# Gryph66/gymwipe

Hardware: AMD Instinct MI355X
Metric: env.step()/s at 65 536 parallel envs, counter-traffic band-assign (higher is better)
Workload: dtype f64

## Files before the change

### gymwipe_amd/csrc/ct_rollout_sfx.hip

```cpp
#include "ct_common.hip.h"
#include "gw_dispatch.h"
#include "gw_queue.h"

using namespace gwk;

namespace {


constexpr int TP_ENVS = 64, TP_STEPS = 64;

__global__ __launch_bounds__(256) void pack_actions_kernel(uint32_t N, int K, int Kp, const int32_t* __restrict__ device,
                                                           const int32_t* __restrict__ duration, uint16_t* __restrict__ packed)
{
    __shared__ __attribute__((aligned(16))) uint16_t tile[TP_ENVS][TP_STEPS + 2];
    const uint32_t e0 = blockIdx.x * TP_ENVS;
    const int t = threadIdx.x;
    const bool vec_ok = (N & 3u) == 0;
    for (int k0 = 0; k0 < Kp; k0 += TP_STEPS) {
        const int c4 = (t & 15) * 4, r = t >> 4;
#pragma unroll
        for (int pass = 0; pass < TP_STEPS / 16; ++pass) {
            const int kk = pass * 16 + r, k = k0 + kk;
            uint32_t v[4] = {0xffffu, 0xffffu, 0xffffu, 0xffffu};
            if (k < K) {
// ... 132 lines not shown
    }
    {
        const int n_tr = (R * R * S + 15) >> 4, n_be = (2 * D * S * 8) >> 4, n_cl = (2 * D * S) >> 4;
        for (int i = threadIdx.x; i < n_tr; i += blockDim.x) *reinterpret_cast<uint4*>(s_trans + ((uint32_t)i << 4)) = ld<uint4>(st.trans, (uint32_t)i << 4);
        for (int i = threadIdx.x; i < n_be; i += blockDim.x) *reinterpret_cast<uint4*>(reinterpret_cast<uint8_t*>(s_ber) + ((uint32_t)i << 4)) = ld<uint4>(st.ber2, (uint32_t)i << 4);
        for (int i = threadIdx.x; i < n_cl; i += blockDim.x) *reinterpret_cast<uint4*>(s_cls + ((uint32_t)i << 4)) = ld<uint4>(st.cls2, (uint32_t)i << 4);
    }
    __syncthreads();
    if (e >= N) return;

    const uint32_t RB = GEN ? (uint32_t)st.RB : 16u * NWC;
    const uint32_t o16 = e << 4, oq = e * RB;
    const uint4 ip = ld<uint4>(st.ip, o16);
    const double2 tw = ld<double2>(st.tw, o16);
    const uint4 tk = ld<uint4>(st.tk, o16);
    typename ArrSel<GEN, DM>::rw len, tb;
    typename ArrSel<GEN, DM + 1>::rw sta;
    if constexpr (GEN) {
        uint32_t* col = s_cols + (threadIdx.x & 63);
        len.p = col; tb.p = col + DM * 64; sta.p = col + 2 * DM * 64;
        for (int i = 0; i < D; ++i) len[i] = st.qb[oq + (uint32_t)i];
        for (int j = 0; j < R; ++j) sta[j] = st.qb[oq + (uint32_t)(D + j)];
    } else {
        uint4 qw[NWC];
#pragma unroll
        for (int w = 0; w < NWC; ++w) qw[w] = ld<uint4>(st.qb, oq + 16u * w);
#pragma unroll
        for (int i = 0; i < DT; ++i) len[i] = (word_of(qw[i >> 4], (i >> 2) & 3) >> ((i & 3) * 8)) & 0xffu;
#pragma unroll
        for (int j = 0; j < DT + 1; ++j) sta[j] = (word_of(qw[(DT + j) >> 4], ((DT + j) >> 2) & 3) >> (((DT + j) & 3) * 8)) & 0xffu;
    }
    double now = tw.x, wake = tw.y;
    uint32_t tau = tk.x;
    const uint32_t nbp = tk.y;
    GwBp bpc, bpp;
    bpc.t0 = ip.x; bpc.c0 = ip.y;
    bpp.t0 = ip.z; bpp.c0 = ip.w;
    const GwBp* hist = st.bph + ((size_t)e << 7);
    uint32_t rvm = tk.z;
    int32_t last_abs = (int32_t)(tk.w & 0x7fffffffu);
    uint32_t dn = tk.w >> 31;

    constexpr bool FAST = MODE >= 1, NOLIM = MODE == 2;
    const StepMathT<FAST, NOLIM> m(c);
    const double slot = c.slot, br = c.bit_rate, hd = c.hdr_dur, hdr_bits = c.hdr_bits, interval = c.counter_interval;
    const double inv_interval = c.inv_interval, tie_filter = c.tie_filter;
    const bool fast_ticks = FAST || c.fast_ticks != 0;
    const uint32_t bound = (uint32_t)c.counter_bound, base_bytes = (uint32_t)(c.mac_hdr + c.net_hdr);
    const int mh = c.mac_hdr, pv = c.payload_value;
    uint32_t live_mask = 0u;
    if constexpr (GEN) {
        for (int i = 0; i < D; ++i) live_mask |= ((s_term[i] >> sta[i]) & 1u) ? 0u : (1u << i);
    }
    typename ArrSel<GEN, DM>::ro mult, term, inv16;
    if constexpr (GEN) {
        mult.p = st.cst->mult; mult.shift16 = 0; term.p = st.cst->term; term.shift16 = 1; inv16.p = st.cst->inv16; inv16.shift16 = 0;
// ... 206 lines not shown
            len_d = gw_len_after_ticks(len_d, kk, mult_d, kt);
        }
    }

    {
        uint32_t kk = 0;
        while (wake <= now) { if (wake == now) fl |= GW_FLAG_TIE; wake = wake + interval; kk++; }
        tau += kk;
#pragma unroll
        for (int i = 0; i < D; ++i) len[i] = gw_len_after_ticks(len[i], tau - tb[i], mult[i], kt);
    }

    if constexpr (GEN) {
        for (int i = 0; i < D; ++i) st.qb[oq + (uint32_t)i] = (uint8_t)len[i];
        for (int j = 0; j < R; ++j) st.qb[oq + (uint32_t)(D + j)] = (uint8_t)sta[j];
    } else {
        uint32_t nb[16 * NWC];
#pragma unroll
        for (int b = 0; b < 16 * NWC; ++b) nb[b] = 0u;
#pragma unroll
        for (int i = 0; i < DT; ++i) nb[i] = len[i];
#pragma unroll
        for (int j = 0; j < DT + 1; ++j) nb[DT + j] = sta[j];
#pragma unroll
        for (int w = 0; w < NWC; ++w) {
            const int b = 16 * w;
            uint4 o;
            o.x = nb[b + 0] | (nb[b + 1] << 8) | (nb[b + 2] << 16) | (nb[b + 3] << 24);
            o.y = nb[b + 4] | (nb[b + 5] << 8) | (nb[b + 6] << 16) | (nb[b + 7] << 24);
            o.z = nb[b + 8] | (nb[b + 9] << 8) | (nb[b + 10] << 16) | (nb[b + 11] << 24);
            o.w = nb[b + 12] | (nb[b + 13] << 8) | (nb[b + 14] << 16) | (nb[b + 15] << 24);
            st_plain(st.qb, oq + 16u * w, o);
        }
    }
    st_plain(st.tw, o16, make_double2(now, wake));
    st_plain(st.tk, o16, make_uint4(tau, nbp, rvm, (uint32_t)last_abs | (dn << 31)));
    publish_env_counters(st.sa, N, e, kt.pop, kt.deliv, k_bad, fl, (uint32_t)K);
}

__device__ __forceinline__ uint32_t gw_policy_u(uint64_t seed, uint64_t env_term, uint64_t step)
{
    uint64_t z = seed ^ env_term ^ (step * 0xD1B54A32D192ED03ull);
    z += 0x9E3779B97F4A7C15ull;
    z = (z ^ (z >> 30)) * 0xBF58476D1CE4E5B9ull;
    z = (z ^ (z >> 27)) * 0x94D049BB133111EBull;
    z ^= z >> 31;
    return gw_min_u32((uint32_t)z, 0xfffffffeu);
}
template <class ROW>
__device__ __forceinline__ uint32_t gw_policy_upper(ROW row, uint32_t A, uint32_t u)
{
// ... 411 lines not shown
```

### gymwipe_amd/csrc/ct_rollout_sync_body.h

```cpp
    constexpr bool GEN = DT == 0;
    constexpr int DM = GEN ? GW_MAX_DEVICES : DT;
    constexpr int NWC = (2 * DM + 1 + 15) / 16;
    constexpr int S = GW_MAX_NSTATES;
    const int D = GEN ? c.D : DT, R = D + 1, RRM = D;
    const uint32_t N = (uint32_t)st.N;
    const uint32_t e = blockIdx.x * blockDim.x + threadIdx.x;

    constexpr int TRANS_B = ((DM + 1) * (DM + 1) * S + 15) / 16 * 16;
    __shared__ __attribute__((aligned(16))) uint8_t s_trans[TRANS_B];
    __shared__ __attribute__((aligned(16))) double  s_ber[2 * DM * S];
    __shared__ __attribute__((aligned(16))) uint8_t s_cls[2 * DM * S];
    __shared__ uint32_t s_cols[GEN ? (3 * DM + 1) * 64 : 1];
    __shared__ uint2 s_mi[GEN ? DM : 1];
    __shared__ uint32_t s_term[GEN ? DM : 1];
    if constexpr (GEN) {
        for (int i = threadIdx.x; i < D; i += blockDim.x) {
            s_mi[i] = make_uint2((uint32_t)st.cst->mult[i], st.cst->inv16[i]);
            s_term[i] = st.cst->term[i];
        }
    }
    {
        const int n_tr = (R * R * S + 15) >> 4, n_be = (2 * D * S * 8) >> 4, n_cl = (2 * D * S) >> 4;
        for (int i = threadIdx.x; i < n_tr; i += blockDim.x) *reinterpret_cast<uint4*>(s_trans + ((uint32_t)i << 4)) = ld<uint4>(st.trans, (uint32_t)i << 4);
        for (int i = threadIdx.x; i < n_be; i += blockDim.x) *reinterpret_cast<uint4*>(reinterpret_cast<uint8_t*>(s_ber) + ((uint32_t)i << 4)) = ld<uint4>(st.ber2, (uint32_t)i << 4);
        for (int i = threadIdx.x; i < n_cl; i += blockDim.x) *reinterpret_cast<uint4*>(s_cls + ((uint32_t)i << 4)) = ld<uint4>(st.cls2, (uint32_t)i << 4);
    }
    GW_ROLLOUT_SRC_STAGE
    __syncthreads();
    if (e >= N) return;

    const uint32_t RB = GEN ? (uint32_t)st.RB : 16u * NWC;
    const uint32_t o16 = e << 4, oq = e * RB;
    const uint4 ip = ld<uint4>(st.ip, o16);
    const double2 tw = ld<double2>(st.tw, o16);
    const uint4 tk = ld<uint4>(st.tk, o16);
    typename ArrSel<GEN, DM>::rw len, tb;
    typename ArrSel<GEN, DM + 1>::rw sta;
    if constexpr (GEN) {
        uint32_t* col = s_cols + (threadIdx.x & 63);
        len.p = col; tb.p = col + DM * 64; sta.p = col + 2 * DM * 64;
        for (int i = 0; i < D; ++i) len[i] = st.qb[oq + (uint32_t)i];
        for (int j = 0; j < R; ++j) sta[j] = st.qb[oq + (uint32_t)(D + j)];
    } else {
        uint4 qw[NWC];
#pragma unroll
        for (int w = 0; w < NWC; ++w) qw[w] = ld<uint4>(st.qb, oq + 16u * w);
#pragma unroll
        for (int i = 0; i < DT; ++i) len[i] = (word_of(qw[i >> 4], (i >> 2) & 3) >> ((i & 3) * 8)) & 0xffu;
#pragma unroll
        for (int j = 0; j < DT + 1; ++j) sta[j] = (word_of(qw[(DT + j) >> 4], ((DT + j) >> 2) & 3) >> (((DT + j) & 3) * 8)) & 0xffu;
    }
    double now = tw.x, wake = tw.y;
    uint32_t tau = tk.x;
    const uint32_t nbp = tk.y;
    GwBp bpc, bpp;
    bpc.t0 = ip.x; bpc.c0 = ip.y;
    bpp.t0 = ip.z; bpp.c0 = ip.w;
    const GwBp* hist = st.bph + ((size_t)e << 7);
    uint32_t rvm = tk.z;
    int32_t last_abs = (int32_t)(tk.w & 0x7fffffffu);
    uint32_t dn = tk.w >> 31;

    constexpr bool FAST = MODE >= 1, NOLIM = MODE == 2;
    const StepMathT<FAST, NOLIM> m(c);
    const double slot = c.slot, br = c.bit_rate, hd = c.hdr_dur, hdr_bits = c.hdr_bits, interval = c.counter_interval;
    const double inv_interval = c.inv_interval, tie_filter = c.tie_filter, coded_factor = c.coded_factor;
    const bool fast_ticks = FAST || c.fast_ticks != 0;
    const bool idem = c.idem_states != 0;
    const uint32_t bound = (uint32_t)c.counter_bound, base_bytes = (uint32_t)(c.mac_hdr + c.net_hdr);
    const int mh = c.mac_hdr, pv = c.payload_value;
    uint32_t live_mask = 0u;
    if constexpr (GEN) {
        for (int i = 0; i < D; ++i) live_mask |= ((s_term[i] >> sta[i]) & 1u) ? 0u : (1u << i);
    }
    typename ArrSel<GEN, DM>::ro mult, term, inv16;
    if constexpr (GEN) {
// ... 237 lines not shown
        uint32_t nb[16 * NWC];
#pragma unroll
        for (int b = 0; b < 16 * NWC; ++b) nb[b] = 0u;
#pragma unroll
        for (int i = 0; i < DT; ++i) nb[i] = len[i];
#pragma unroll
        for (int j = 0; j < DT + 1; ++j) nb[DT + j] = sta[j];
#pragma unroll
        for (int w = 0; w < NWC; ++w) {
            const int b = 16 * w;
            uint4 o;
            o.x = nb[b + 0] | (nb[b + 1] << 8) | (nb[b + 2] << 16) | (nb[b + 3] << 24);
            o.y = nb[b + 4] | (nb[b + 5] << 8) | (nb[b + 6] << 16) | (nb[b + 7] << 24);
            o.z = nb[b + 8] | (nb[b + 9] << 8) | (nb[b + 10] << 16) | (nb[b + 11] << 24);
            o.w = nb[b + 12] | (nb[b + 13] << 8) | (nb[b + 14] << 16) | (nb[b + 15] << 24);
            st_plain(st.qb, oq + 16u * w, o);
        }
    }
    st_plain(st.tw, o16, make_double2(now, wake));
    st_plain(st.tk, o16, make_uint4(tau, nbp, rvm, (uint32_t)last_abs | (dn << 31)));
    publish_env_counters(st.sa, N, e, kt.pop, kt.deliv, k_bad, fl, (uint32_t)K);
```

### gymwipe_amd/csrc/ct_step_sfx.hip

```cpp
#include "ct_common.hip.h"
#include "gw_dispatch.h"
#include "gw_queue.h"

using namespace gwk;


namespace {



#define PIN_V(x) asm volatile("" : "+v"(x))
#define PIN_S(x) asm volatile("" : "+s"(x))

template <int DT, bool FEEDBACK, int MODE, bool HALF = false>
__device__ __forceinline__ void ct_step_sfx_body(const GwState& st, const GwDevConst& c,
                                                 const int32_t* __restrict__ device,
                                                 const int32_t* __restrict__ duration,
                                                 int32_t* __restrict__ obs,
                                                 float* __restrict__ reward,
                                                 uint8_t* __restrict__ done,
                                                 uint8_t* __restrict__ fb,
                                                 int n_stage,
                                                 double& now_out, bool& live_out)
{
    constexpr bool PACKED = DT > 0;
    constexpr bool FAST = MODE >= 1, NOLIM = MODE == 2;
    constexpr int NWC = DT > 0 ? (2 * DT + 1 + 15) / 16 : 1;
    const uint32_t N = (uint32_t)st.N;
    const uint32_t e = HALF ? blockIdx.x * 32u + (threadIdx.x & 31u) : blockIdx.x * 64u + threadIdx.x;
    const int D = DT > 0 ? DT : c.D;
    const int R = D + 1, RRM = D;
    constexpr int S = GW_MAX_NSTATES;
    const uint32_t RB = PACKED ? 16u * NWC : (uint32_t)st.RB;

    STAMP(0);
    constexpr int DM = DT > 0 ? DT : GW_MAX_DEVICES;
    constexpr GwStripeLayout LM(DM);
    const GwStripeLayout L(D);
    constexpr int MAX_CH = LM.staged_chunks(GW_MAX_NSTATES);
    const int n_ch = n_stage < MAX_CH ? n_stage : MAX_CH;
    const int tid = threadIdx.x;
    constexpr int nthr = 64;
// ... 9 lines not shown
            r_ch[i] = ld<uint4>(st.blob, (uint32_t)(ch < n_ch ? ch : 0) << 4);
        }
    }

    Tally k = {0, 0, 0, 0, 0};
    uint32_t k_bad = 0;

    const bool live = e < N && (!HALF || threadIdx.x < 32u);
    const uint32_t el = live ? e : 0u;
    const uint32_t o16 = e << 4, o16l = el << 4;
    const uint32_t oq = e * RB, oql = el * RB;
    int d = device[el];
    int du = duration[el];
    uint4 ip = ld<uint4>(st.ip, o16l);
    const double2 tw = ld<double2>(st.tw, o16l);
    const uint4 tk = ld<uint4>(st.tk, o16l);
    uint4 qw[NWC];
#pragma unroll
    for (int w = 0; w < NWC; ++w) qw[w] = PACKED ? ld<uint4>(st.qb, oql + 16u * w) : make_uint4(0u, 0u, 0u, 0u);
    now_out = tw.x;
    live_out = live;
    if (one_pass) {
#pragma unroll
        for (int i = 0; i < PER; ++i) {
            const int ch = tid + i * nthr;
            *reinterpret_cast<uint4*>(s_blob + ((uint32_t)ch << 4)) = r_ch[i];
        }
    } else {
        for (int i = tid; i < n_ch; i += nthr) *reinterpret_cast<uint4*>(s_blob + ((uint32_t)i << 4)) = ld<uint4>(st.blob, (uint32_t)i << 4);
    }
    STAMP(1);
// ... 16 lines not shown
    PIN_V(d); PIN_V(du);
    PIN_V(ip.x); PIN_V(ip.y); PIN_V(ip.z); PIN_V(ip.w);
    const uint2* s_mi = reinterpret_cast<const uint2*>(s_blob + L.mi);
    const uint8_t* s_st = s_blob + L.s0;
    const uint8_t* g_h2 = st.blob + L.h2;
    const uint32_t STR = (uint32_t)L.stripe, DD = (uint32_t)D;
    auto t_ber0 = [&](uint32_t dd, uint32_t ss) { return *reinterpret_cast<const double*>(s_st + ss * STR + (uint32_t)L.ber0 + dd * 8u); };
    auto t_ber1 = [&](uint32_t dd, uint32_t ss) { return *reinterpret_cast<const double*>(s_st + ss * STR + (uint32_t)L.ber1 + dd * 8u); };
    auto t_h1 = [&](uint32_t j, uint32_t ss) { return (uint32_t)s_st[ss * STR + (uint32_t)L.h1 + j]; };
    auto t_r1 = [&](uint32_t dd, uint32_t ss) { return (uint32_t)s_st[ss * STR + (uint32_t)L.r1 + dd]; };
    auto t_cls0 = [&](uint32_t dd, uint32_t ss) { return (uint32_t)s_st[ss * STR + (uint32_t)L.cls0 + dd]; };
    auto t_cls1 = [&](uint32_t dd, uint32_t ss) { return (uint32_t)s_st[ss * STR + (uint32_t)L.cls1 + dd]; };
    auto t_h2 = [&](uint32_t j, uint32_t dd, uint32_t ss) { return (uint32_t)g_h2[(ss * DD + j) * DD + dd]; };

    if (live) {
        uint32_t rvm = tk.z;
#ifdef GW_STAMPS
        asm volatile("" : "+v"(rvm));
#endif
        STAMP(3);
        int32_t last_abs = (int32_t)(tk.w & 0x7fffffffu);
        uint32_t dn = tk.w >> 31;
        uint32_t fl = 0;

        if ((unsigned)d >= (unsigned)D || (unsigned)du >= (unsigned)max_duration) {
            fl = GW_FLAG_BADACT;
            k_bad = 1;
            const int32_t latest = pv * ((int)(rvm & 1u) - (int)((rvm >> 1) & 1u));
            if (FEEDBACK) {
                obs[e] = latest + cbound;
                reward[e] = 0.0f;
                done[e] = (uint8_t)dn;
                if (fb) fb[e] = (uint8_t)((uint32_t)(((latest > 0) - (latest < 0)) + 1) | (10u << 2) | (dn << 7));
            }
        } else {
            const uint32_t bound = (uint32_t)cbound;
            const uint32_t base_bytes = (uint32_t)base_b;
// ... 15 lines not shown
                        const bool hl = ((uint32_t)d >> 4) == (uint32_t)w, hs = ((uint32_t)(DT + d) >> 4) == (uint32_t)w;
                        lx = hl ? q0 : lx; ly = hl ? q1 : ly; lz = hl ? q2 : lz; lw = hl ? q3 : lw;
                        sx = hs ? q0 : sx; sy = hs ? q1 : sy; sz = hs ? q2 : sz; sw = hs ? q3 : sw;
                    }
                    len_d = byte_of(lx, ly, lz, lw, (uint32_t)d & 15u);
                    s_d_old = byte_of(sx, sy, sz, sw, (uint32_t)(DT + d) & 15u);
                }
                s_r_old = (word_of(qw[(2 * DT) >> 4], ((2 * DT) >> 2) & 3) >> (((2 * DT) & 3) * 8)) & 0xffu;
            } else {
                len_d = st.qb[oq + (uint32_t)d];
                s_d_old = st.qb[oq + (uint32_t)(D + d)];
                s_r_old = st.qb[oq + (uint32_t)(2 * D)];
            }
            const double t_a = tw.x;
            double wake = tw.y;
            const uint32_t tau0 = tk.x, nbp = tk.y;
            GwBp bpc, bpp;
            bpc.t0 = ip.x; bpc.c0 = ip.y;
            bpp.t0 = ip.z; bpp.c0 = ip.w;
            const GwBp* hist = st.bph + ((size_t)e << 7);
            const uint32_t s_d = t_h1((uint32_t)d, s_d_old);
            const uint32_t s_r1 = t_r1((uint32_t)d, s_r_old);
            const uint2 mi = s_mi[d];
            uint32_t nb[PACKED ? 16 * NWC : 1];
            uint32_t n1[PACKED ? DT : 1], n2[PACKED ? DT : 1], mlt[PACKED ? DT : 1];
            if (PACKED) {
#pragma unroll
                for (int b = 0; b < 16 * NWC; ++b) nb[b] = (word_of(qw[b >> 4], (b >> 2) & 3) >> ((b & 3) * 8)) & 0xffu;
#pragma unroll
                for (int i = 0; i < DT; ++i) {
                    n1[i] = t_h1((uint32_t)i, nb[DT + i]);
// ... 116 lines not shown
                    k.deliv += okx ? pops : 0u;
                    rvm |= okx ? (1u << d) : 0u;
                    dn = (okx && pv == cbound) ? 1u : dn;
                }
                if (more)
                for (;;) {
                    if (len_d == 0) {
                        if (mult_d != 0u && wake < stopw) {
                            cur = wake;
                            wake = wake + interval;
                            tau++;
                            len_d = gw_len_after_ticks(0u, 1u, mult_d, kd);
                        } else break;
                    }
                    const uint32_t age = gw_ceil_div(len_d, mult_d, inv16_d);
                    const uint32_t s = base_bytes + gw_tick_value(tau - age, bpc, bpp, nbp, hist, bound);
                    const double need = m.over_rate((double)(s * 8u));
                    if (!((stopw - cur) > need)) break;
                    len_d--;
                    k.pop++;
                    const int pay = (int)s - mh;
                    const TxTimes x = tx_times(m, cur, hd, m.over_rate((double)(pay * 8)));
                    k.tx++;
                    n_data++;
                    double ber_x = ber_x1;
                    uint32_t cls_x = cls_x1;
                    if (idem) {
                        s_r = s_r1;
                    } else {
                        s_r = st.trans[(uint32_t)((RRM * R + d) * S) + s_r];
                        ber_x = st.ber[(uint32_t)((RRM * R + d) * S) + s_r];
// ... 24 lines not shown
                return s;
            };
            if (PACKED) {
                const uint32_t heard_data = n_data ? 0xffffffffu : 0u;
#pragma unroll
                for (int i = 0; i < DT; ++i) {
                    Tally ki = {0, 0, 0, 0, 0};
                    const uint32_t li = gw_len_after_ticks(nb[i], n_ticks, mlt[i], ki);
                    uint32_t si = (n2[i] & heard_data) | (n1[i] & ~heard_data);
                    if (!idem) si = heard_slow(i, nb[DT + i]);
                    if (i != d) { k.app += ki.app; k.drop += ki.drop; }
                    nb[i] = (i == d) ? len_d : li;
                    nb[DT + i] = (i == d) ? s_d : si;
                }
                nb[2 * DT] = s_r;
                uint4 o[NWC];
#pragma unroll
                for (int w = 0; w < NWC; ++w) {
                    const int b = 16 * w;
                    o[w].x = nb[b + 0] | (nb[b + 1] << 8) | (nb[b + 2] << 16) | (nb[b + 3] << 24);
                    o[w].y = nb[b + 4] | (nb[b + 5] << 8) | (nb[b + 6] << 16) | (nb[b + 7] << 24);
                    o[w].z = nb[b + 8] | (nb[b + 9] << 8) | (nb[b + 10] << 16) | (nb[b + 11] << 24);
                    o[w].w = nb[b + 12] | (nb[b + 13] << 8) | (nb[b + 14] << 16) | (nb[b + 15] << 24);
                }
                STAMP(9);
#pragma unroll
                for (int w = 0; w < NWC; ++w) st_(st.qb, oq + 16u * w, o[w]);
            } else {
                for (int i = 0; i < D; ++i) {
                    if (i == d) continue;
                    const uint32_t l0 = st.qb[oq + (uint32_t)i];
                    const uint32_t s0 = st.qb[oq + (uint32_t)(D + i)];
                    const uint32_t s1 = !idem ? heard_slow(i, s0)
                                              : (n_data ? t_h2((uint32_t)i, (uint32_t)d, s0) : t_h1((uint32_t)i, s0));
                    st.qb[oq + (uint32_t)i] = (uint8_t)gw_len_after_ticks(l0, n_ticks, s_mi[i].x, k);
                    if (s1 != s0) st.qb[oq + (uint32_t)(D + i)] = (uint8_t)s1;
                }
                st.qb[oq + (uint32_t)d] = (uint8_t)len_d;
// ... 4 lines not shown
            STAMP(10);
            const int32_t latest = pv * ((int)(rvm & 1u) - (int)((rvm >> 1) & 1u));
            const int32_t abs_d = latest < 0 ? -latest : latest;
            int32_t r = last_abs - abs_d;
            last_abs = abs_d;
            r = r > 10 ? 10 : (r < -10 ? -10 : r);
            if (FEEDBACK) {
                st_(obs, e << 2, (int32_t)(latest + cbound));
                st_(reward, e << 2, (float)r);
                st_(done, e, (uint8_t)dn);
                if (fb) st_(fb, e, (uint8_t)((uint32_t)(((latest > 0) - (latest < 0)) + 1) | ((uint32_t)(r + 10) << 2) | (dn << 7)));
            }
            now_out = t_end;

            st_(st.tw, o16, make_double2(t_end, wake));
            st_(st.tk, o16, make_uint4(tau, nbp, rvm, (uint32_t)last_abs | (dn << 31)));
        }
        STAMP(11);
        publish_env_counters(st.sa, N, e, k.pop, k.deliv, k_bad, fl, 1u);
    }
    STAMP(12);
}

template <int DT, int MODE>
__global__ __launch_bounds__(64) void ct_step_sfx_kernel(GW_LEAD_PARAMS_U64, uint64_t obs_a, uint64_t reward_a, uint64_t done_a, uint64_t fb_a)
{
    uint32_t* __restrict__ ip = gw_global_at<uint32_t>(ip_a);
    double* __restrict__ tw = gw_global_at<double>(tw_a);
    uint32_t* __restrict__ tk = gw_global_at<uint32_t>(tk_a);
    uint8_t* __restrict__ qb = gw_global_at<uint8_t>(qb_a);
    const int32_t* __restrict__ device = gw_global_at<const int32_t>(device_a);
// ... 131 lines not shown
    for (int w = 0; w < GW_SA_WORDS; ++w) st.sa[(size_t)w * st.N + e] = 0u;
    if (e == 0u) { st.sa[(size_t)4 * st.N] = 0u; st.sa[(size_t)4 * st.N + 1] = 0u; }
}

__global__ void ct_reset_sfx_kernel(uint32_t* __restrict__ ip, uint32_t n_envs, uint32_t n_dev, const uint8_t* __restrict__ mask,
                                    int32_t* __restrict__ obs)
{
    const uint32_t e = blockIdx.x * blockDim.x + threadIdx.x;
    if (e >= n_envs) return;
    const uint8_t* base = reinterpret_cast<const uint8_t*>(ip) - gw_blob_header((int)n_dev);
    const GW_AS_CONST GwState* hs = (const GW_AS_CONST GwState*)(base + gw_hdr_st_off((int)n_dev));
    uint32_t* tkp = gw_as_global(hs->tk);
    GwBp* bph = gw_as_global(hs->bph);
    const GW_AS_CONST GwDevConst* c = (const GW_AS_CONST GwDevConst*)(base + gw_hdr_cst_off((int)n_dev));
    const uint32_t o16 = e << 4;
    uint32_t rvm;
    if (!mask || mask[e]) {
        uint4 tk = ld<uint4>(tkp, o16);
        uint4 bp = ld<uint4>(ip, o16);
        GwBp cur; cur.t0 = bp.x; cur.c0 = 0u;
        if (bp.x == tk.x) {
            bph[((size_t)e << 7) + ((tk.y - 1u) & GW_RING_MASK)] = cur;
            bp.y = 0u;
        } else {
            bp.z = bp.x; bp.w = bp.y;
            cur.t0 = tk.x;
            bph[((size_t)e << 7) + (tk.y & GW_RING_MASK)] = cur;
            tk.y += 1u; bp.x = cur.t0; bp.y = 0u;
        }
        tk.z = 0u; tk.w = 0u;
        st_(tkp, o16, tk);
        st_(ip, o16, bp);
        rvm = 0u;
    } else {
        rvm = ld<uint4>(tkp, o16).z;
    }
    if (obs) obs[e] = c->payload_value * ((int)(rvm & 1u) - (int)((rvm >> 1) & 1u)) + c->counter_bound;
}

__global__ void ct_received_sfx_kernel(GwState st, int32_t* __restrict__ out)
{
    const int64_t idx = (int64_t)blockIdx.x * blockDim.x + threadIdx.x;
    const int D = st.D;
    if (idx >= st.N * D) return;
    const uint32_t e = (uint32_t)(idx / D);
    const int i = (int)(idx - (int64_t)e * D);
    const uint32_t rvm = ld<uint4>(st.tk, e << 4).z;
    out[idx] = ((rvm >> i) & 1u) ? st.cst->payload_value : 0;
}

__global__ void ct_delivered_sfx_kernel(GwState st, uint32_t* __restrict__ out)
{
    const uint32_t e = blockIdx.x * blockDim.x + threadIdx.x;
    if (e < (uint32_t)st.N) out[e] = st.sa[(size_t)2 * e + 1];
}

__global__ void ct_clear_flags_kernel(GwState st)
{
    const int64_t e = (int64_t)blockIdx.x * blockDim.x + threadIdx.x;
    if (e < st.N) {
        if (st.sa) st.sa[(size_t)3 * st.N + e] = 0u;
        if (st.xc) st.xc[(size_t)e * 4 + 3] = 0u;
// ... 118 lines not shown
```

### gymwipe_amd/csrc/gw_api.cpp

```cpp
#include "gw_internal.h"
#include "gw_queue.h"
#include "gw_runq.h"
#include "gw_fastmath.h"

#include <hip/hip_runtime.h>

#include <math.h>
#include <stdarg.h>
#include <stdio.h>
#include <stdlib.h>
#include <string.h>
#include <new>
#include <vector>
#include <deque>
#include <atomic>
#include <string>

namespace {

thread_local char g_err[512] = "";

int fail(int code, const char* fmt, ...)
{
    va_list ap;
// ... 210 lines not shown
    for (int j = 0; j < R; ++j) {
        uint16_t m = 0;
        for (int s0 = 0; s0 < tab.nstates[j]; ++s0) {
            bool fixed = true;
            for (int f = 0; f < R && fixed; ++f)
                if (f != j && tab.trans[((size_t)j * R + f) * GW_MAX_NSTATES + s0] != s0) fixed = false;
            if (fixed) m |= (uint16_t)(1u << s0);
        }
        k.term[j] = m;
    }
    return GW_OK;
}

int gw_validate_config(const gw_config& cfg) { return validate(cfg); }

struct GwEnvCounts { std::vector<uint64_t> steps, tx, deliv, app, pop, drop, bad; std::vector<uint32_t> flags; };
static int derive_env_counts(gw_env* env, GwEnvCounts& c)
{
    const GwState& st = env->st;
    const int64_t N = st.N;
    const int D = st.D, RB = st.RB;
    std::vector<uint32_t> sa((size_t)N * GW_SA_WORDS + 2), tk((size_t)N * 4);
    std::vector<uint8_t> qb((size_t)N * RB);
    HIP_TRY(hipMemcpy(sa.data(), st.sa, sa.size() * sizeof(uint32_t), hipMemcpyDeviceToHost));
    HIP_TRY(hipMemcpy(tk.data(), st.tk, tk.size() * sizeof(uint32_t), hipMemcpyDeviceToHost));
    HIP_TRY(hipMemcpy(qb.data(), st.qb, qb.size(), hipMemcpyDeviceToHost));
    uint64_t mult_sum = 0;
    for (int i = 0; i < D; ++i) mult_sum += (uint64_t)env->cfg.mult[i];
    const uint64_t n_steps = (uint64_t)sa[(size_t)4 * N] | ((uint64_t)sa[(size_t)4 * N + 1] << 32);
    c.steps.resize(N); c.tx.resize(N); c.deliv.resize(N); c.app.resize(N); c.pop.resize(N); c.drop.resize(N); c.bad.resize(N);
    c.flags.resize(N);
    for (int64_t e = 0; e < N; ++e) {
        uint64_t queued = 0;
        for (int i = 0; i < D; ++i) queued += qb[(size_t)e * RB + i];
        c.pop[e] = sa[(size_t)2 * e];
        c.deliv[e] = sa[(size_t)2 * e + 1];
        c.bad[e] = sa[(size_t)2 * N + e];
        c.flags[e] = sa[(size_t)3 * N + e];
        c.steps[e] = n_steps - c.bad[e];
        c.tx[e] = c.steps[e] + c.pop[e];
        c.app[e] = (uint64_t)tk[(size_t)e * 4] * mult_sum;
// ... 560 lines not shown
int gw_now_ptr(gw_env* env, const void** now_dev, int64_t* stride_bytes)
{
    if (!env || !now_dev || !stride_bytes) return fail(GW_EINVAL, "env/now/stride is NULL");
    if (env->st.tw) { *now_dev = env->st.tw; *stride_bytes = 16; }
    else { *now_dev = env->st.xw; *stride_bytes = 16; }
    return GW_OK;
}

struct GwSnapHeader {
    uint32_t magic, abi;
    uint64_t total;
    gw_config cfg;
    int32_t nblocks, dyn;
    uint64_t block_bytes[32];
    double t_bound;
    int32_t captured, pad;
};
static const uint32_t kSnapMagic = 0x4e535747u;

int gw_snapshot_bytes(gw_env* env, uint64_t* bytes)
{
    if (!env || !bytes) return fail(GW_EINVAL, "env/bytes is NULL");
    uint64_t t = sizeof(GwSnapHeader);
    for (int i = 0; i < env->nblocks_create; ++i) t += env->block_bytes[i];
    *bytes = t;
    return GW_OK;
}

int gw_get_snapshot(gw_env* env, void* dst, uint64_t bytes)
{
    if (!env || !dst) return fail(GW_EINVAL, "env/dst is NULL");
    uint64_t need = 0;
    int rc = gw_snapshot_bytes(env, &need);
    if (rc) return rc;
    if (bytes != need) return fail(GW_EINVAL, "snapshot needs %llu bytes, got %llu", (unsigned long long)need, (unsigned long long)bytes);
    if ((rc = select_device(env))) return rc;
    HIP_TRY(hipDeviceSynchronize());
    GwSnapHeader h;
    memset(&h, 0, sizeof h);
    h.magic = kSnapMagic; h.abi = GW_ABI_VERSION; h.total = need; h.cfg = env->cfg; h.nblocks = env->nblocks_create; h.dyn = env->dyn;
    for (int i = 0; i < env->nblocks_create; ++i) h.block_bytes[i] = env->block_bytes[i];
    h.t_bound = env->t_bound;
    h.captured = env->captured;
    uint8_t* o = (uint8_t*)dst;
    memcpy(o, &h, sizeof h);
    o += sizeof h;
    for (int i = 0; i < env->nblocks_create; ++i) {
        HIP_TRY(hipMemcpy(o, env->blocks[i], env->block_bytes[i], hipMemcpyDeviceToHost));
        o += env->block_bytes[i];
    }
    return GW_OK;
}

int gw_set_state(gw_env* env, const void* src, uint64_t bytes)
{
    if (!env || !src) return fail(GW_EINVAL, "env/src is NULL");
    uint64_t need = 0;
    int rc = gw_snapshot_bytes(env, &need);
    if (rc) return rc;
    if (bytes != need) return fail(GW_EINVAL, "a snapshot of this handle has %llu bytes, got %llu", (unsigned long long)need, (unsigned long long)bytes);
    GwSnapHeader h;
    memcpy(&h, src, sizeof h);
    if (h.magic != kSnapMagic || h.abi != (uint32_t)GW_ABI_VERSION || h.total != bytes) return fail(GW_EINVAL, "not a snapshot of this ABI");
    gw_config a = h.cfg, b = env->cfg;
    a.hip_device = b.hip_device = 0;
    if (memcmp(&a, &b, sizeof a) != 0 || h.nblocks != env->nblocks_create || h.dyn != env->dyn)
        return fail(GW_EINVAL, "snapshot belongs to a handle with another configuration");
    for (int i = 0; i < h.nblocks; ++i)
        if (h.block_bytes[i] != env->block_bytes[i]) return fail(GW_EINVAL, "snapshot belongs to a handle with another layout");
    if ((rc = select_device(env))) return rc;
    HIP_TRY(hipDeviceSynchronize());
    const uint8_t* in = (const uint8_t*)src + sizeof h;
    for (int i = 0; i < h.nblocks; ++i) {
        HIP_TRY(hipMemcpy(env->blocks[i], in, env->block_bytes[i], hipMemcpyHostToDevice));
        in += env->block_bytes[i];
    }
    if (env->st.ip && (rc = upload_header_structs(env))) return rc;
    env->t_bound = h.t_bound > env->t_bound ? h.t_bound : env->t_bound;
    env->captured |= h.captured;
    HIP_TRY(hipDeviceSynchronize());
    return GW_OK;
}
// ... 282 lines not shown
                    if (k == 5) { NEED(N, uint32_t); memcpy(dst, c.flags.data(), bytes); return GW_OK; }
                    NEED(N, uint64_t);
                    const std::vector<uint64_t>& v = k == 0 ? c.tx : (k == 1 ? c.deliv : (k == 2 ? c.app : (k == 3 ? c.pop : c.drop)));
                    memcpy(dst, v.data(), bytes);
                    return GW_OK;
                }
        }
        const int RB = st.RB;
        std::vector<double> tw((size_t)N * 2);
        std::vector<uint32_t> tk((size_t)N * 4), ip((size_t)N * 4);
        std::vector<uint8_t> qb((size_t)N * RB);
        HIP_TRY(hipMemcpy(tw.data(), st.tw, tw.size() * sizeof(double), hipMemcpyDeviceToHost));
        HIP_TRY(hipMemcpy(tk.data(), st.tk, tk.size() * sizeof(uint32_t), hipMemcpyDeviceToHost));
        HIP_TRY(hipMemcpy(ip.data(), st.ip, ip.size() * sizeof(uint32_t), hipMemcpyDeviceToHost));
        HIP_TRY(hipMemcpy(qb.data(), st.qb, qb.size(), hipMemcpyDeviceToHost));
        const uint32_t bound = (uint32_t)env->cfg.counter_bound;
        const int pv = env->cfg.payload_value;
        if (!strcmp(field, "now")) { NEED(N, double); double* o = (double*)dst; for (int64_t e = 0; e < N; ++e) o[e] = tw[e * 2]; return GW_OK; }
        if (!strcmp(field, "wake")) {
            NEED(N * D, double); double* o = (double*)dst;
            for (int64_t e = 0; e < N; ++e) for (int i = 0; i < D; ++i) o[e * D + i] = tw[e * 2 + 1];
            return GW_OK;
        }
        if (!strcmp(field, "counter")) {
            NEED(N * D, uint32_t); uint32_t* o = (uint32_t*)dst;
            for (int64_t e = 0; e < N; ++e) {
                const uint32_t v = gw_min_u32(ip[e * 4 + 1] + (tk[e * 4] - ip[e * 4]), bound);
                for (int i = 0; i < D; ++i) o[e * D + i] = v;
            }
            return GW_OK;
// ... 148 lines not shown
```

### gymwipe_amd/csrc/gw_queue.h

```cpp
#pragma once
#include <stdint.h>
#include "gw_internal.h"

#if defined(__HIPCC__)
#include <hip/hip_runtime.h>
#define GW_HD __host__ __device__ __forceinline__
#else
#define GW_HD inline
#endif

struct GwTally { uint32_t app, pop, drop, tx, deliv; };

GW_HD uint32_t gw_min_u32(uint32_t a, uint32_t b) { return a < b ? a : b; }

GW_HD uint32_t gw_ceil_div(uint32_t len, uint32_t mult, uint32_t inv16)
{
    return ((len + mult - 1u) * inv16) >> 16;
}

GW_HD uint32_t gw_tick_value(uint32_t t, GwBp cur, GwBp prev, uint32_t nbp, const GwBp* hist, uint32_t bound)
{
    const bool older = t < cur.t0;
    GwBp b;
    b.t0 = older ? prev.t0 : cur.t0;
    b.c0 = older ? prev.c0 : cur.c0;
    if (older && t < prev.t0) {
        uint32_t j = nbp - 2u;
        do { --j; b = hist[j & GW_RING_MASK]; } while (t < b.t0);
    }
    return gw_min_u32(b.c0 + (t - b.t0), bound);
}

GW_HD uint32_t gw_len_after_ticks(uint32_t len, uint32_t k, uint32_t mult, GwTally& t)
{
    const uint32_t add = k * mult;
    const uint32_t want = len + add;
    const uint32_t now = gw_min_u32(want, (uint32_t)GW_QUEUE_CAP);
    t.app += add;
    t.drop += want - now;
    return now;
}
```

Before: 17.49 billion.

## Pack hot per-env tick state into unused queue-record tail bytes

```diff
diff --git a/gymwipe_amd/csrc/ct_rollout_sfx.hip b/gymwipe_amd/csrc/ct_rollout_sfx.hip
--- a/gymwipe_amd/csrc/ct_rollout_sfx.hip
+++ b/gymwipe_amd/csrc/ct_rollout_sfx.hip
@@ -170,6 +170,12 @@
     const uint4 ip = ld<uint4>(st.ip, o16);
     const double2 tw = ld<double2>(st.tw, o16);
     const uint4 tk = ld<uint4>(st.tk, o16);
+    const bool hot_tail = GEN ? gw_hot_tail(true, D) : gw_hot_tail(true, DT);
+    GwHot hot = {tk.x, tk.z, tk.w >> 31, (int32_t)(tk.w & 0x7fffffffu)};
+    if (hot_tail) {
+        const uint4 qt = ld<uint4>(st.qb, oq + RB - 16u);
+        hot = gw_tail_unpack(D, qt.y, qt.z, qt.w, c.payload_value);
+    }
     typename ArrSel<GEN, DM>::rw len, tb;
     typename ArrSel<GEN, DM + 1>::rw sta;
     if constexpr (GEN) {
@@ -187,15 +193,15 @@
         for (int j = 0; j < DT + 1; ++j) sta[j] = (word_of(qw[(DT + j) >> 4], ((DT + j) >> 2) & 3) >> (((DT + j) & 3) * 8)) & 0xffu;
     }
     double now = tw.x, wake = tw.y;
-    uint32_t tau = tk.x;
+    uint32_t tau = hot.tau;
     const uint32_t nbp = tk.y;
     GwBp bpc, bpp;
     bpc.t0 = ip.x; bpc.c0 = ip.y;
     bpp.t0 = ip.z; bpp.c0 = ip.w;
     const GwBp* hist = st.bph + ((size_t)e << 7);
-    uint32_t rvm = tk.z;
-    int32_t last_abs = (int32_t)(tk.w & 0x7fffffffu);
-    uint32_t dn = tk.w >> 31;
+    uint32_t rvm = hot.rvm;
+    int32_t last_abs = hot.last_abs;
+    uint32_t dn = hot.dn;
 
     constexpr bool FAST = MODE >= 1, NOLIM = MODE == 2;
     const StepMathT<FAST, NOLIM> m(c);
@@ -432,6 +438,14 @@
     if constexpr (GEN) {
         for (int i = 0; i < D; ++i) st.qb[oq + (uint32_t)i] = (uint8_t)len[i];
         for (int j = 0; j < R; ++j) st.qb[oq + (uint32_t)(D + j)] = (uint8_t)sta[j];
+        if (hot_tail) {
+            uint32_t ty = 0u, tz = 0u, tw_ = 0u;
+            gw_tail_pack(D, ty, tz, tw_, tau, rvm, dn, last_abs);
+            const uint64_t tyz = ((uint64_t)tz << 32) | ty;
+            const int nfb = gw_tail_flag_bytes(D);
+            for (int b = 0; b < nfb; ++b) st.qb[oq + RB - 4u - (uint32_t)(nfb - b)] = (uint8_t)(tyz >> (8 * (8 - nfb + b)));
+            st_plain(st.qb, oq + RB - 4u, tw_);
+        }
     } else {
         uint32_t nb[16 * NWC];
 #pragma unroll
@@ -448,11 +462,12 @@
             o.y = nb[b + 4] | (nb[b + 5] << 8) | (nb[b + 6] << 16) | (nb[b + 7] << 24);
             o.z = nb[b + 8] | (nb[b + 9] << 8) | (nb[b + 10] << 16) | (nb[b + 11] << 24);
             o.w = nb[b + 12] | (nb[b + 13] << 8) | (nb[b + 14] << 16) | (nb[b + 15] << 24);
+            if (hot_tail && w == NWC - 1) gw_tail_pack(DT, o.y, o.z, o.w, tau, rvm, dn, last_abs);
             st_plain(st.qb, oq + 16u * w, o);
         }
     }
     st_plain(st.tw, o16, make_double2(now, wake));
-    st_plain(st.tk, o16, make_uint4(tau, nbp, rvm, (uint32_t)last_abs | (dn << 31)));
+    if (!hot_tail) st_plain(st.tk, o16, make_uint4(tau, nbp, rvm, (uint32_t)last_abs | (dn << 31)));
     publish_env_counters(st.sa, N, e, kt.pop, kt.deliv, k_bad, fl, (uint32_t)K);
 }
 
diff --git a/gymwipe_amd/csrc/ct_rollout_sync_body.h b/gymwipe_amd/csrc/ct_rollout_sync_body.h
--- a/gymwipe_amd/csrc/ct_rollout_sync_body.h
+++ b/gymwipe_amd/csrc/ct_rollout_sync_body.h
@@ -34,6 +34,8 @@
     const uint4 ip = ld<uint4>(st.ip, o16);
     const double2 tw = ld<double2>(st.tw, o16);
     const uint4 tk = ld<uint4>(st.tk, o16);
+    constexpr bool HOT = gw_hot_tail(true, DT);
+    GwHot hot = {tk.x, tk.z, tk.w >> 31, (int32_t)(tk.w & 0x7fffffffu)};
     typename ArrSel<GEN, DM>::rw len, tb;
     typename ArrSel<GEN, DM + 1>::rw sta;
     if constexpr (GEN) {
@@ -49,17 +51,18 @@
         for (int i = 0; i < DT; ++i) len[i] = (word_of(qw[i >> 4], (i >> 2) & 3) >> ((i & 3) * 8)) & 0xffu;
 #pragma unroll
         for (int j = 0; j < DT + 1; ++j) sta[j] = (word_of(qw[(DT + j) >> 4], ((DT + j) >> 2) & 3) >> (((DT + j) & 3) * 8)) & 0xffu;
+        if constexpr (HOT) hot = gw_tail_unpack(DT, qw[NWC - 1].y, qw[NWC - 1].z, qw[NWC - 1].w, c.payload_value);
     }
     double now = tw.x, wake = tw.y;
-    uint32_t tau = tk.x;
+    uint32_t tau = hot.tau;
     const uint32_t nbp = tk.y;
     GwBp bpc, bpp;
     bpc.t0 = ip.x; bpc.c0 = ip.y;
     bpp.t0 = ip.z; bpp.c0 = ip.w;
     const GwBp* hist = st.bph + ((size_t)e << 7);
-    uint32_t rvm = tk.z;
-    int32_t last_abs = (int32_t)(tk.w & 0x7fffffffu);
-    uint32_t dn = tk.w >> 31;
+    uint32_t rvm = hot.rvm;
+    int32_t last_abs = hot.last_abs;
+    uint32_t dn = hot.dn;
 
     constexpr bool FAST = MODE >= 1, NOLIM = MODE == 2;
     const StepMathT<FAST, NOLIM> m(c);
@@ -327,9 +330,10 @@
             o.y = nb[b + 4] | (nb[b + 5] << 8) | (nb[b + 6] << 16) | (nb[b + 7] << 24);
             o.z = nb[b + 8] | (nb[b + 9] << 8) | (nb[b + 10] << 16) | (nb[b + 11] << 24);
             o.w = nb[b + 12] | (nb[b + 13] << 8) | (nb[b + 14] << 16) | (nb[b + 15] << 24);
+            if constexpr (HOT) { if (w == NWC - 1) gw_tail_pack(DT, o.y, o.z, o.w, tau, rvm, dn, last_abs); }
             st_plain(st.qb, oq + 16u * w, o);
         }
     }
     st_plain(st.tw, o16, make_double2(now, wake));
-    st_plain(st.tk, o16, make_uint4(tau, nbp, rvm, (uint32_t)last_abs | (dn << 31)));
+    if constexpr (!HOT) st_plain(st.tk, o16, make_uint4(tau, nbp, rvm, (uint32_t)last_abs | (dn << 31)));
     publish_env_counters(st.sa, N, e, kt.pop, kt.deliv, k_bad, fl, (uint32_t)K);
diff --git a/gymwipe_amd/csrc/ct_step_sfx.hip b/gymwipe_amd/csrc/ct_step_sfx.hip
--- a/gymwipe_amd/csrc/ct_step_sfx.hip
+++ b/gymwipe_amd/csrc/ct_step_sfx.hip
@@ -26,6 +26,7 @@
     constexpr bool PACKED = DT > 0;
     constexpr bool FAST = MODE >= 1, NOLIM = MODE == 2;
     constexpr int NWC = DT > 0 ? (2 * DT + 1 + 15) / 16 : 1;
+    constexpr bool HOT = gw_hot_tail(true, DT);
     const uint32_t N = (uint32_t)st.N;
     const uint32_t e = HALF ? blockIdx.x * 32u + (threadIdx.x & 31u) : blockIdx.x * 64u + threadIdx.x;
     const int D = DT > 0 ? DT : c.D;
@@ -65,7 +66,7 @@
     int du = duration[el];
     uint4 ip = ld<uint4>(st.ip, o16l);
     const double2 tw = ld<double2>(st.tw, o16l);
-    const uint4 tk = ld<uint4>(st.tk, o16l);
+    const uint4 tk = HOT ? make_uint4(0u, 0u, 0u, 0u) : ld<uint4>(st.tk, o16l);
     uint4 qw[NWC];
 #pragma unroll
     for (int w = 0; w < NWC; ++w) qw[w] = PACKED ? ld<uint4>(st.qb, oql + 16u * w) : make_uint4(0u, 0u, 0u, 0u);
@@ -112,13 +113,15 @@
     auto t_h2 = [&](uint32_t j, uint32_t dd, uint32_t ss) { return (uint32_t)g_h2[(ss * DD + j) * DD + dd]; };
 
     if (live) {
-        uint32_t rvm = tk.z;
+        GwHot hot = {0u, 0u, 0u, 0};
+        if constexpr (HOT) hot = gw_tail_unpack(DT, qw[NWC - 1].y, qw[NWC - 1].z, qw[NWC - 1].w, pv);
+        uint32_t rvm = HOT ? hot.rvm : tk.z;
 #ifdef GW_STAMPS
         asm volatile("" : "+v"(rvm));
 #endif
         STAMP(3);
-        int32_t last_abs = (int32_t)(tk.w & 0x7fffffffu);
-        uint32_t dn = tk.w >> 31;
+        int32_t last_abs = HOT ? hot.last_abs : (int32_t)(tk.w & 0x7fffffffu);
+        uint32_t dn = HOT ? hot.dn : tk.w >> 31;
         uint32_t fl = 0;
 
         if ((unsigned)d >= (unsigned)D || (unsigned)du >= (unsigned)max_duration) {
@@ -164,7 +167,7 @@
             }
             const double t_a = tw.x;
             double wake = tw.y;
-            const uint32_t tau0 = tk.x, nbp = tk.y;
+            const uint32_t tau0 = HOT ? hot.tau : tk.x, nbp = tk.y;
             GwBp bpc, bpp;
             bpc.t0 = ip.x; bpc.c0 = ip.y;
             bpp.t0 = ip.z; bpp.c0 = ip.w;
@@ -311,7 +314,8 @@
                         } else break;
                     }
                     const uint32_t age = gw_ceil_div(len_d, mult_d, inv16_d);
-                    const uint32_t s = base_bytes + gw_tick_value(tau - age, bpc, bpp, nbp, hist, bound);
+                    const uint32_t s = base_bytes + (HOT ? gw_tick_value_lazy(tau - age, bpc, bpp, st.tk + ((size_t)e << 2) + 1, hist, bound)
+                                                         : gw_tick_value(tau - age, bpc, bpp, nbp, hist, bound));
                     const double need = m.over_rate((double)(s * 8u));
                     if (!((stopw - cur) > need)) break;
                     len_d--;
@@ -366,6 +370,10 @@
                     nb[DT + i] = (i == d) ? s_d : si;
                 }
                 nb[2 * DT] = s_r;
+                if (HOT) {
+#pragma unroll
+                    for (int b = 2 * DT + 1; b < 16 * NWC; ++b) nb[b] = 0u;
+                }
                 uint4 o[NWC];
 #pragma unroll
                 for (int w = 0; w < NWC; ++w) {
@@ -374,6 +382,10 @@
                     o[w].y = nb[b + 4] | (nb[b + 5] << 8) | (nb[b + 6] << 16) | (nb[b + 7] << 24);
                     o[w].z = nb[b + 8] | (nb[b + 9] << 8) | (nb[b + 10] << 16) | (nb[b + 11] << 24);
                     o[w].w = nb[b + 12] | (nb[b + 13] << 8) | (nb[b + 14] << 16) | (nb[b + 15] << 24);
+                }
+                if constexpr (HOT) {
+                    const int32_t abs_new = pv * (int)((rvm ^ (rvm >> 1)) & 1u);
+                    gw_tail_pack(DT, o[NWC - 1].y, o[NWC - 1].z, o[NWC - 1].w, tau, rvm, dn, abs_new);
                 }
                 STAMP(9);
 #pragma unroll
@@ -408,7 +420,7 @@
             now_out = t_end;
 
             st_(st.tw, o16, make_double2(t_end, wake));
-            st_(st.tk, o16, make_uint4(tau, nbp, rvm, (uint32_t)last_abs | (dn << 31)));
+            if (!HOT) st_(st.tk, o16, make_uint4(tau, nbp, rvm, (uint32_t)last_abs | (dn << 31)));
         }
         STAMP(11);
         publish_env_counters(st.sa, N, e, k.pop, k.deliv, k_bad, fl, 1u);
@@ -570,9 +582,16 @@
     GwBp* bph = gw_as_global(hs->bph);
     const GW_AS_CONST GwDevConst* c = (const GW_AS_CONST GwDevConst*)(base + gw_hdr_cst_off((int)n_dev));
     const uint32_t o16 = e << 4;
+    const bool hot = gw_hot_tail(hs->rxp == nullptr, (int)n_dev);
+    uint8_t* qbp = gw_as_global(hs->qb);
+    const uint32_t oqt = e * (uint32_t)gw_rec_bytes((int)n_dev) + (uint32_t)gw_rec_bytes((int)n_dev) - 16u;
+    uint4 qt = make_uint4(0u, 0u, 0u, 0u);
+    if (hot) qt = ld<uint4>(qbp, oqt);
+    const GwHot h = gw_tail_unpack((int)n_dev, qt.y, qt.z, qt.w, c->payload_value);
     uint32_t rvm;
     if (!mask || mask[e]) {
         uint4 tk = ld<uint4>(tkp, o16);
+        if (hot) tk.x = h.tau;
         uint4 bp = ld<uint4>(ip, o16);
         GwBp cur; cur.t0 = bp.x; cur.c0 = 0u;
         if (bp.x == tk.x) {
@@ -585,11 +604,16 @@
             tk.y += 1u; bp.x = cur.t0; bp.y = 0u;
         }
         tk.z = 0u; tk.w = 0u;
+        if (hot) {
+            tk.x = 0u;
+            gw_tail_pack((int)n_dev, qt.y, qt.z, qt.w, h.tau, 0u, 0u, 0);
+            st_(qbp, oqt, qt);
+        }
         st_(tkp, o16, tk);
         st_(ip, o16, bp);
         rvm = 0u;
     } else {
-        rvm = ld<uint4>(tkp, o16).z;
+        rvm = hot ? h.rvm : ld<uint4>(tkp, o16).z;
     }
     if (obs) obs[e] = c->payload_value * ((int)(rvm & 1u) - (int)((rvm >> 1) & 1u)) + c->counter_bound;
 }
@@ -601,7 +625,13 @@
     if (idx >= st.N * D) return;
     const uint32_t e = (uint32_t)(idx / D);
     const int i = (int)(idx - (int64_t)e * D);
-    const uint32_t rvm = ld<uint4>(st.tk, e << 4).z;
+    uint32_t rvm;
+    if (gw_hot_tail(st.rxp == nullptr, D)) {
+        const uint4 qt = ld<uint4>(st.qb, e * (uint32_t)st.RB + (uint32_t)st.RB - 16u);
+        rvm = gw_tail_unpack(D, qt.y, qt.z, qt.w, 0).rvm;
+    } else {
+        rvm = ld<uint4>(st.tk, e << 4).z;
+    }
     out[idx] = ((rvm >> i) & 1u) ? st.cst->payload_value : 0;
 }
 
diff --git a/gymwipe_amd/csrc/gw_api.cpp b/gymwipe_amd/csrc/gw_api.cpp
--- a/gymwipe_amd/csrc/gw_api.cpp
+++ b/gymwipe_amd/csrc/gw_api.cpp
@@ -248,6 +248,22 @@
 
 int gw_validate_config(const gw_config& cfg) { return validate(cfg); }
 
+static bool env_hot_tail(const gw_env* env) { return gw_hot_tail(env->st.tk != nullptr && !env->dyn, env->st.D); }
+static void canonical_tk(const gw_env* env, std::vector<uint32_t>& tk, const std::vector<uint8_t>& qb)
+{
+    if (!env_hot_tail(env)) return;
+    const int64_t N = env->st.N;
+    const int RB = env->st.RB;
+    for (int64_t e = 0; e < N; ++e) {
+        uint32_t t3[3];
+        memcpy(t3, &qb[(size_t)e * RB + RB - 12], sizeof t3);
+        const GwHot h = gw_tail_unpack(env->st.D, t3[0], t3[1], t3[2], env->cfg.payload_value);
+        tk[(size_t)e * 4] = h.tau;
+        tk[(size_t)e * 4 + 2] = h.rvm;
+        tk[(size_t)e * 4 + 3] = (uint32_t)h.last_abs | (h.dn << 31);
+    }
+}
+
 struct GwEnvCounts { std::vector<uint64_t> steps, tx, deliv, app, pop, drop, bad; std::vector<uint32_t> flags; };
 static int derive_env_counts(gw_env* env, GwEnvCounts& c)
 {
@@ -259,6 +275,7 @@
     HIP_TRY(hipMemcpy(sa.data(), st.sa, sa.size() * sizeof(uint32_t), hipMemcpyDeviceToHost));
     HIP_TRY(hipMemcpy(tk.data(), st.tk, tk.size() * sizeof(uint32_t), hipMemcpyDeviceToHost));
     HIP_TRY(hipMemcpy(qb.data(), st.qb, qb.size(), hipMemcpyDeviceToHost));
+    canonical_tk(env, tk, qb);
     uint64_t mult_sum = 0;
     for (int i = 0; i < D; ++i) mult_sum += (uint64_t)env->cfg.mult[i];
     const uint64_t n_steps = (uint64_t)sa[(size_t)4 * N] | ((uint64_t)sa[(size_t)4 * N + 1] << 32);
@@ -849,7 +866,8 @@
     int32_t nblocks, dyn;
     uint64_t block_bytes[32];
     double t_bound;
-    int32_t captured, pad;
+    int32_t captured;
+    int32_t hot_tail;
 };
 static const uint32_t kSnapMagic = 0x4e535747u;
 
@@ -877,6 +895,7 @@
     for (int i = 0; i < env->nblocks_create; ++i) h.block_bytes[i] = env->block_bytes[i];
     h.t_bound = env->t_bound;
     h.captured = env->captured;
+    h.hot_tail = env_hot_tail(env) ? 1 : 0;
     uint8_t* o = (uint8_t*)dst;
     memcpy(o, &h, sizeof h);
     o += sizeof h;
@@ -901,6 +920,7 @@
     a.hip_device = b.hip_device = 0;
     if (memcmp(&a, &b, sizeof a) != 0 || h.nblocks != env->nblocks_create || h.dyn != env->dyn)
         return fail(GW_EINVAL, "snapshot belongs to a handle with another configuration");
+    if (h.hot_tail != (env_hot_tail(env) ? 1 : 0)) return fail(GW_EINVAL, "snapshot belongs to a handle with another record format");
     for (int i = 0; i < h.nblocks; ++i)
         if (h.block_bytes[i] != env->block_bytes[i]) return fail(GW_EINVAL, "snapshot belongs to a handle with another layout");
     if ((rc = select_device(env))) return rc;
@@ -1213,6 +1233,7 @@
         HIP_TRY(hipMemcpy(tk.data(), st.tk, tk.size() * sizeof(uint32_t), hipMemcpyDeviceToHost));
         HIP_TRY(hipMemcpy(ip.data(), st.ip, ip.size() * sizeof(uint32_t), hipMemcpyDeviceToHost));
         HIP_TRY(hipMemcpy(qb.data(), st.qb, qb.size(), hipMemcpyDeviceToHost));
+        canonical_tk(env, tk, qb);
         const uint32_t bound = (uint32_t)env->cfg.counter_bound;
         const int pv = env->cfg.payload_value;
         if (!strcmp(field, "now")) { NEED(N, double); double* o = (double*)dst; for (int64_t e = 0; e < N; ++e) o[e] = tw[e * 2]; return GW_OK; }
diff --git a/gymwipe_amd/csrc/gw_queue.h b/gymwipe_amd/csrc/gw_queue.h
--- a/gymwipe_amd/csrc/gw_queue.h
+++ b/gymwipe_amd/csrc/gw_queue.h
@@ -31,6 +31,54 @@
     return gw_min_u32(b.c0 + (t - b.t0), bound);
 }
 
+GW_HD uint32_t gw_tick_value_lazy(uint32_t t, GwBp cur, GwBp prev, const uint32_t* nbp_at, const GwBp* hist, uint32_t bound)
+{
+    const bool older = t < cur.t0;
+    GwBp b;
+    b.t0 = older ? prev.t0 : cur.t0;
+    b.c0 = older ? prev.c0 : cur.c0;
+    if (older && t < prev.t0) {
+        uint32_t j = *nbp_at - 2u;
+        do { --j; b = hist[j & GW_RING_MASK]; } while (t < b.t0);
+    }
+    return gw_min_u32(b.c0 + (t - b.t0), bound);
+}
+
+constexpr int gw_rec_bytes(int D) { return 16 * ((2 * D + 1 + 15) / 16); }
+constexpr int gw_tail_flag_bytes(int D) { return (D + 2 + 7) / 8; }
+constexpr int gw_tail_bytes(int D) { return 4 + gw_tail_flag_bytes(D); }
+constexpr bool gw_hot_tail_fits(int D)
+{
+    constexpr int dts[] = {GW_DTS_STEP};
+    bool listed = false;
+    for (int dt : dts) listed = listed || dt == D;
+    return listed && 2 * D + 1 + gw_tail_bytes(D) <= gw_rec_bytes(D);
+}
+constexpr bool gw_hot_tail(bool table_phy_sfx, int D) { return table_phy_sfx && gw_hot_tail_fits(D); }
+
+struct GwHot { uint32_t tau, rvm, dn; int32_t last_abs; };
+
+GW_HD GwHot gw_tail_unpack(int D, uint32_t y, uint32_t z, uint32_t w, int32_t payload_value)
+{
+    const int sh = 8 * (8 - gw_tail_flag_bytes(D));
+    const uint64_t f = (((uint64_t)z << 32) | y) >> sh;
+    GwHot h;
+    h.tau = w;
+    h.rvm = (uint32_t)f & (D >= 32 ? 0xffffffffu : ((1u << D) - 1u));
+    h.dn = (uint32_t)(f >> D) & 1u;
+    h.last_abs = ((f >> (D + 1)) & 1u) ? (payload_value < 0 ? -payload_value : payload_value) : 0;
+    return h;
+}
+GW_HD void gw_tail_pack(int D, uint32_t& y, uint32_t& z, uint32_t& w, uint32_t tau, uint32_t rvm, uint32_t dn, int32_t last_abs)
+{
+    const int sh = 8 * (8 - gw_tail_flag_bytes(D));
+    const uint64_t f = (uint64_t)rvm | ((uint64_t)(dn & 1u) << D) | ((uint64_t)(last_abs != 0) << (D + 1));
+    const uint64_t yz = ((((uint64_t)z << 32) | y) & ((1ull << sh) - 1ull)) | (f << sh);
+    y = (uint32_t)yz;
+    z = (uint32_t)(yz >> 32);
+    w = tau;
+}
+
 GW_HD uint32_t gw_len_after_ticks(uint32_t len, uint32_t k, uint32_t mult, GwTally& t)
 {
     const uint32_t add = k * mult;
```

New measurement: 16.82 billion. -3.8%, worse.
